# orottier/web-audio-api-rs

Measured on NVIDIA H100. Metric: offline render-quanta/sec (48kHz stereo, 128-frame), higher is better.
Workload: dtype f64 filter state / f32 PCM

## Files before the change

web-audio-api-rs_b200/csrc/wae_engine.cu:

```cuda
#include "wae_graph.h"
#include "wae_hostmath.h"
#include "wae_hrtf_host.h"
#include "wae_resample_host.h"
#include "wae_kernels.h"
#include "wae_param_core.h"
#include "wae_param_host.h"

#include <cuda_runtime.h>
#include <emmintrin.h>

#include <algorithm>
#include <atomic>
#include <chrono>
#include <condition_variable>
#include <cstdlib>
#include <deque>
#include <fstream>
#include <mutex>
#include <sched.h>
#include <sstream>
#include <thread>
#include <cmath>
#include <cstdio>
#include <cstring>
// ... 576 lines not shown
    Node* n = nullptr;
    int level = 0;
    std::vector<std::vector<PortRef>> in_edges;
    std::vector<int> in_ch;
    std::vector<BufRef> in_buf;
    std::vector<Lay> in_lay;
    std::vector<int> out_ch;
    std::vector<BufRef> out_buf;
    std::vector<Lay> out_lay;
    bool wrote_dest = false;
    Lay lay_out(int port) const { return port < (int)out_lay.size() ? out_lay[port] : Lay::fixed(out_ch[port]); }
};

struct NodeTable {
    std::vector<PNode> v;
    std::vector<char> has;
    void reset(uint32_t max_id) {
        if (v.size() < (size_t)max_id + 1) v.resize((size_t)max_id + 1);
        has.assign(v.size(), 0);
    }
    PNode& put(uint32_t id, Node* n) {
        if (id >= v.size()) {
            v.resize((size_t)id + 1);
            has.resize((size_t)id + 1, 0);
        }
        PNode& p = v[id];
        p.n = n;
        p.level = 0;
        p.in_edges.resize((size_t)n->n_inputs);
        for (auto& port : p.in_edges) port.clear();
        p.in_ch.clear();
        p.in_buf.clear();
        p.in_lay.clear();
        p.out_ch.clear();
        p.out_buf.clear();
        p.out_lay.clear();
        p.wrote_dest = false;
        has[id] = 1;
        return p;
    }
    PNode* find(uint32_t id) { return id < v.size() && has[id] ? &v[id] : nullptr; }
    bool count(uint32_t id) const { return id < v.size() && has[id]; }
    PNode& at(uint32_t id) {
        if (!(id < v.size() && has[id])) throw std::out_of_range("planner: unknown node id");
        return v[id];
    }
};

struct Planner {
    wae_batch* b;
    wae_engine* eng;
    std::map<std::pair<int, int>, StageBuild> builds;
    std::string error;
    int error_code = 0;
    uint64_t algorithmic_bytes = 0;
    struct IrSpectra {
        float2* h;
        int S;
        int channels;
    };
    std::unordered_map<uint64_t, IrSpectra> own_ir_cache;
    std::unordered_map<uint64_t, IrSpectra>* ir_cache = &own_ir_cache;
    std::map<int, std::pair<const float2*, const float2*>> os_filters;

    bool has_feedback = false;
    std::map<std::pair<uint32_t, uint32_t>, int>* delay_ch_hint = nullptr;
    std::map<std::pair<uint32_t, uint32_t>, int> delay_ch_seen;
    struct DelayRing {
        float* ring;
        uint32_t ring_len;
        int ch;
        int64_t* mono_at;
        int32_t mono_len;
    };
    std::map<std::pair<uint32_t, uint32_t>, DelayRing> delay_rings;
    std::map<std::pair<uint32_t, uint32_t>, int> conv_paths_seen;
    bool dry = false;
    int group_graphs = 1;
    int vs_mode = -1;
    int voice_sum_mode() {
        if (eng->voice_sum >= 0) return eng->voice_sum;
        if (vs_mode < 0) {
            const char* e = getenv("WAE_VOICE_SUM");
            vs_mode = e ? std::max(0, std::min(2, atoi(e))) : 0;
        }
        return vs_mode;
    }
    uint64_t arena_floats_per_frame = 0;
    float* d_src = nullptr;
    std::vector<wae_batch::Group::SrcCopy>* src_copies = nullptr;
    size_t src_cursor = 0;
    struct PendingChain {
        ChainInst inst;
        hm::BiquadCoefs coefs[CHAIN_MAX_BIQUADS] = {};
        int ch = 1;
        int phase = 0;
        int cls = 0;
        Lay lay;
    };

    uint32_t key_graph = 0, key_node = 0, key_seq = 0;
    uint64_t key_salt = 0;
    template <typename T>
    T* alloc(size_t count, bool zero = false, bool rezero_on_run = false) {
        if (dry) return reinterpret_cast<T*>(uintptr_t(256));
        if (seg_start == 0 && seg_end >= lq) return b->dalloc<T>(count, zero, rezero_on_run);
        const wae_batch::StateKey key{key_graph, key_node, key_seq++, key_salt};
        const size_t bytes = count * sizeof(T);
        std::lock_guard<std::recursive_mutex> lk(b->mu);
        auto it = b->state_map.find(key);
        if (it != b->state_map.end() && it->second.second == bytes) return (T*)it->second.first;
        T* p = b->dalloc<T>(count, zero, rezero_on_run);
        if (p) b->state_map[key] = {(void*)p, bytes};
        return p;
    }
    std::map<int, std::vector<float*>> arena_pool;
    std::map<int, size_t> arena_used;
    std::map<std::pair<uint32_t, uint32_t>, size_t> src_offsets;
    std::unordered_map<const PcmBuffer*, size_t> buf_offsets;
    struct ParamRecord {
        size_t n_source_events = 0;
        ParamTimeline tl;
        int64_t init_frame = 0;
    };
    std::unordered_map<uint64_t, ParamRecord> param_records;
    const ParamTimeline* param_timeline(uint32_t gi, uint32_t pid, const Param& prm, float sample_rate) {
        const uint64_t rec_key = (uint64_t)gi << 32 | pid;
        auto it = param_records.find(rec_key);
        if (it == param_records.end()) {
            ParamRecord r;
            r.tl = build_param_timeline(prm);
            r.n_source_events = prm.events.size();
            r.init_frame = seg_start;
            return &param_records.emplace(rec_key, std::move(r)).first->second.tl;
        }
        ParamRecord& r = it->second;
        if (r.n_source_events == prm.events.size() || !r.tl.error.empty()) return &r.tl;
        ParamInst host{};
        host.events = r.tl.events.data();
        host.curves = r.tl.curves.data();
        host.n_events = (int32_t)r.tl.events.size();
        host.a_rate = prm.a_rate ? 1 : 0;
        host.sample_rate = sample_rate;
        ParamState st{};
        st.intrinsic = r.tl.intrinsic;
        st.has_last = r.tl.has_last ? 1 : 0;
        st.last = r.tl.last;
        st.inited = 1;
        float buf[128];
        for (int64_t f = r.init_frame; f < seg_start; f += 128) param_compute_buffer(host, st, (double)f / (double)sample_rate, buf);
        ParamTimeline next;
        next.curves = r.tl.curves;
        for (int i = st.head; i < host.n_events; i++) next.events.push_back(i == st.head && st.override_valid ? st.override_ev : r.tl.events[i]);
        next.intrinsic = st.intrinsic;
        next.has_last = st.has_last != 0;
        next.last = st.last;
        fold_param_events(next, prm.events.data() + r.n_source_events, prm.events.size() - r.n_source_events);
        r.tl = std::move(next);
        r.n_source_events = prm.events.size();
        r.init_frame = seg_start;
        return &r.tl;
    }
    int64_t seg_start = 0, seg_end = 0;
    int64_t lq = 0, glq = 0;
    BufRef dest_ref(const wae_graph* g, uint32_t gi) const { return BufRef{b->d_out + b->out_off[gi], (uint32_t)g->length, 1}; }
    void begin_segment(int64_t f0, int64_t f1) {
        seg_start = f0;
// ... 593 lines not shown
                    m.n_edges = (int)edges.size();
                    m.edge_offset = (uint32_t)ms.mix_edges.size();
                    m.limit = -1;
                    for (auto& r : edges) ms.mix_edges.push_back(MixEdge{pn.at(r.node).out_buf[r.port], pn.at(r.node).out_ch[r.port], 0});
                    ms.mix_dyn.push_back(m);
                    pi.in = m.out;
                } else {
                    StageBuild& ms = stage(2 * level, S_MIX);
                    MixInst m{};
                    m.out = arena_buf(1);
                    if (!m.out.p) return bail(WAE_OUT_OF_MEMORY, "out of device memory (arena)");
                    m.out_ch = 1;
                    m.interp = WAE_INTERPRETATION_DISCRETE;
                    m.n_edges = (int)edges.size();
                    m.edge_offset = (uint32_t)ms.mix_edges.size();
                    m.limit = -1;
                    for (auto& r : edges) ms.mix_edges.push_back(MixEdge{pn.at(r.node).out_buf[r.port], pn.at(r.node).out_ch[r.port], 0});
                    ms.mix.push_back(m);
                    pi.in = m.out;
                }
            }
            pi.events = tl.events.empty() ? nullptr : upload(tl.events);
            pi.curves = tl.curves.empty() ? nullptr : upload(tl.curves);
            pi.state = alloc<ParamState>(1, true, true);
            pi.out = arena_buf(2);
            if (!pi.state || !pi.out.p) return bail(WAE_OUT_OF_MEMORY, "out of device memory (param)");
            pi.def = n.param.default_value;
            pi.mn = n.param.min_value;
            pi.mx = n.param.max_value;
            pi.intrinsic0 = tl.intrinsic;
            pi.has_last0 = tl.has_last ? 1 : 0;
            pi.last0 = tl.last;
            pi.sample_rate = g->sample_rate;
            pi.n_events = (int32_t)tl.events.size();
            pi.a_rate = n.param.a_rate ? 1 : 0;
            stage(2 * level + 1, S_PARAM).param.push_back(pi);
            p.out_ch = {1};
            p.out_buf = {pi.out};
            continue;
        }
        int level = 0;
        for (auto& port : p.in_edges)
            for (auto& r : port) level = std::max(level, pn.at(r.node).level + 1);
        bool dyn_params = false;
        for (uint32_t pid : n.params) {
            PNode& pp = pn.at(pid);
            if (!pp.out_buf.empty()) {
                dyn_params = true;
                level = std::max(level, pp.level + 1);
            }
        }
        if (n.kind == K_PANNER)
            for (uint32_t pid = 2; pid <= 10; pid++)
                if (pn.count(pid) && !pn.at(pid).out_buf.empty()) level = std::max(level, pn.at(pid).level + 1);
        p.level = level;
        const bool fuse_n = fuse && !dyn_params;
        uint32_t fuse_src = 0;
        bool extend = false, dest_direct = false;
        const bool chain_kind = !dyn_params && ((n.kind == K_BIQUAD && !eng->serial_filters) || (fuse && (n.kind == K_GAIN || (n.kind == K_SHAPER && !(n.oversample && n.has_curve)))));
        if (fuse && n.n_inputs == 1 && p.in_edges[0].size() == 1 && p.in_edges[0][0].port == 0) {
            auto it = pending.find(p.in_edges[0][0].node);
            if (it != pending.end()) {
                int sch = pn.at(it->first).out_ch[0];
                if (chain_kind && computed_channels(n.cfg, sch) == sch && chain_accepts(it->second, n.kind)) {
                    extend = true;
                    fuse_src = it->first;
                } else if (n.kind == K_DEST && g->length <= 0xffffffffull &&
                           (sch == (int)g->channels || (sch == 1 && g->channels == 2 && n.cfg.interp == WAE_INTERPRETATION_SPEAKERS))) {
                    dest_direct = true;
                    fuse_src = it->first;
                }
            }
        }
        std::vector<char> port_vsum(p.in_edges.size(), 0);
        std::vector<int> port_vsum_nb(p.in_edges.size(), 0);
        if (fuse && voice_sum_mode() != 0 && !extend && !dest_direct && cur_cls == 0 && n.kind != K_DELAY_R) {
            for (size_t pi = 0; pi < p.in_edges.size() && (int)pi < n.n_inputs; pi++) {
                const auto& edges = p.in_edges[pi];
                if ((int)edges.size() < 8) continue;
                const int ch = computed_channels(n.cfg, 1);
                if (!(ch == 1 || (ch == 2 && n.cfg.interp == WAE_INTERPRETATION_SPEAKERS))) continue;
                if (n.kind == K_DEST && g->length > 0xffffffffull) continue;
                const int64_t tiles = (seg_end - seg_start + 2047) / 2048;
                if (voice_sum_mode() < 2 && tiles * (int64_t)group_graphs < 2 * (int64_t)voice_sum_slots()) continue;
                int nb = -1;
                bool ok = true;
                std::set<uint32_t> seen_nodes;
                for (auto& r : edges) {
                    auto it = pending.find(r.node);
                    if (r.port != 0 || it == pending.end()) { ok = false; break; }
                    const PendingChain& pc = it->second;
                    if (pc.inst.src_kind != CHAIN_SRC_OSC || pc.ch != 1 || pc.inst.has_shaper || pc.inst.n_biquad > 1 || pc.lay.dyn() || pc.cls != cur_cls ||
                        (nb >= 0 && nb != pc.inst.n_biquad) || !seen_nodes.insert(r.node).second) { ok = false; break; }
                    nb = pc.inst.n_biquad;
                }
                if (!ok) continue;
                port_vsum[pi] = 1;
                port_vsum_nb[pi] = nb;
            }
        }
        for (size_t pi = 0; pi < p.in_edges.size(); pi++) {
            if (port_vsum[pi]) continue;
            auto& port = p.in_edges[pi];
            for (auto& r : port)
                if (!((extend || dest_direct) && r.node == fuse_src))
                    if (!materialize(r.node, n.kind == K_CONV && n.buffer && port.size() == 1)) return false;
        }
        p.in_ch.assign(n.n_inputs, 1);
        p.in_buf.assign(n.n_inputs, BufRef{nullptr, 0, 0});
        p.in_lay.assign(n.n_inputs, Lay::fixed(1));
        for (int port = 0; port < n.n_inputs; port++) {
            auto& edges = p.in_edges[port];
            int max_in = 1;
            for (auto& r : edges) max_in = std::max(max_in, pn.at(r.node).out_ch[r.port]);
            int ch = computed_channels(n.cfg, max_in);
            if (n.kind == K_DELAY_R) {
                ch = max_in;
            }
            p.in_ch[port] = ch;
            p.in_lay[port] = Lay::fixed(ch);
            bool is_dest = n.kind == K_DEST;
            if (extend || dest_direct) {
                if (extend) p.in_lay[port] = pending.at(fuse_src).lay;
                continue;
            }
            if (port_vsum[port]) {
                StageBuild& vs = stage(2 * level, S_VSUM, port_vsum_nb[port]);
                VoiceGroup vg{};
                vg.first = (int32_t)vs.chain.size();
                vg.n_voices = (int32_t)edges.size();
                vg.out_dup = ch;
                vg.limit = -1;
                if (is_dest) {
                    vg.out = dest_ref(g, gi);
                    vg.limit = (int64_t)g->length;
                } else {
                    vg.out = arena_buf(ch);
                    if (!vg.out.p) return bail(WAE_OUT_OF_MEMORY, "out of device memory (arena)");
                }
                for (auto& r : edges) {
                    PendingChain pc = std::move(pending.at(r.node));
                    pending.erase(r.node);
                    if (pc.inst.n_biquad == 1 && vs.n_scan_coef != vs.chain.size()) return bail(WAE_UNSUPPORTED, "internal: voice-sum coefficient table out of step");
                    for (int k = 0; k < pc.inst.n_biquad; k++)
                        pc.inst.bq[k].coef = vs.add_scan_coef(want_scan_coefs, [&] { return make_scan_coef(pc.coefs[k]); });
                    pc.inst.limit = -1;
                    pc.inst.out_dup = 0;
                    vs.chain.push_back(pc.inst);
                }
                vs.vgroups.push_back(vg);
                p.in_buf[port] = vg.out;
                continue;
            }
            if (is_dest && edges.size() == 1 && pn.at(edges[0].node).wrote_dest) {
                p.in_buf[port] = pn.at(edges[0].node).out_buf[edges[0].port];
                continue;
            }
            bool any_dyn = false;
            Lay pl = Lay::fixed(ch);
            if (!edges.empty()) {
                int lo = 1, hi = 1, on_nlo = 0, min_nlo = 255;
                bool all_may_silent = true;
                for (auto& r : edges) {
                    const Lay el = pn.at(r.node).lay_out(r.port);
                    any_dyn = any_dyn || el.dyn();
                    lo = std::max<int>(lo, el.lo);
                    hi = std::max<int>(hi, el.hi);
// ... 1149 lines not shown
    CUDA_TRY(cudaStreamCreateWithFlags(&eng->s_d2h, cudaStreamNonBlocking));
    if (const char* e = getenv("WAE_BIND_NUMA"))
        if (atoi(e) != 0) bind_to_device_numa_node(eng);
    std::vector<float> sine = hm::sine_table();
    CUDA_TRY(cudaMalloc(&eng->d_sine, sine.size() * sizeof(float)));
    CUDA_TRY(cudaMemcpy(eng->d_sine, sine.data(), sine.size() * sizeof(float), cudaMemcpyHostToDevice));
    upload_twiddles();
    CUDA_TRY(cudaDeviceSynchronize());
    *out = eng;
    return WAE_OK;
}

WAE_API wae_status wae_engine_destroy(wae_engine* eng) {
    if (!eng) return WAE_OK;
    cudaSetDevice(eng->device);
    if (eng->d_sine) cudaFree(eng->d_sine);
    if (eng->d_sphere_ir) cudaFree(eng->d_sphere_ir);
    if (eng->d_sphere_pos) cudaFree(eng->d_sphere_pos);
    if (eng->d_sphere_tri) cudaFree(eng->d_sphere_tri);
    eng->drop_rate_spheres();
    delete eng->sphere;
    delete eng->pool;
    eng->dev_trim();
    for (int i = 0; i < wae_engine::kStageSlots; i++)
        if (eng->h_stage[i]) cudaFreeHost(eng->h_stage[i]);
    if (eng->h_ring) cudaFreeHost(eng->h_ring);
    if (eng->stream) cudaStreamDestroy(eng->stream);
    if (eng->s_h2d) cudaStreamDestroy(eng->s_h2d);
    if (eng->s_d2h) cudaStreamDestroy(eng->s_d2h);
    delete eng;
    return WAE_OK;
}

WAE_API wae_status wae_engine_set_hrir_sphere(wae_engine* eng, const void* data, uint64_t len) {
    if (!eng) return fail(WAE_INVALID_ARGUMENT, "null engine");
    auto* sp = new HrirSphere();
    std::string err;
    if (!sp->parse(static_cast<const uint8_t*>(data), len, err)) {
        delete sp;
        return fail(WAE_INVALID_ARGUMENT, err.c_str());
    }
    CUDA_TRY(cudaSetDevice(eng->device));
    float* d = nullptr;
    if (cudaMalloc(&d, sp->ir.size() * sizeof(float)) != cudaSuccess) {
        delete sp;
        return fail(WAE_OUT_OF_MEMORY, "out of device memory (HRIR sphere)");
    }
    float* dpos = nullptr;
    uint32_t* dtri = nullptr;
    if (cudaMalloc(&dpos, sp->pos.size() * sizeof(float)) != cudaSuccess || cudaMalloc(&dtri, sp->tri.size() * sizeof(uint32_t)) != cudaSuccess) {
        cudaFree(d);
        if (dpos) cudaFree(dpos);
        delete sp;
        return fail(WAE_OUT_OF_MEMORY, "out of device memory (HRIR sphere)");
    }
    cudaMemcpy(d, sp->ir.data(), sp->ir.size() * sizeof(float), cudaMemcpyHostToDevice);
    cudaMemcpy(dpos, sp->pos.data(), sp->pos.size() * sizeof(float), cudaMemcpyHostToDevice);
    cudaMemcpy(dtri, sp->tri.data(), sp->tri.size() * sizeof(uint32_t), cudaMemcpyHostToDevice);
    CUDA_TRY(cudaStreamSynchronize(eng->stream));
    if (eng->d_sphere_ir) cudaFree(eng->d_sphere_ir);
    if (eng->d_sphere_pos) cudaFree(eng->d_sphere_pos);
    if (eng->d_sphere_tri) cudaFree(eng->d_sphere_tri);
    eng->drop_rate_spheres();
    eng->d_sphere_pos = dpos;
    eng->d_sphere_tri = dtri;
    delete eng->sphere;
    eng->sphere = sp;
    eng->d_sphere_ir = d;
    return WAE_OK;
}

WAE_API wae_status wae_engine_stream(wae_engine* eng, void** out_stream) {
    *out_stream = (void*)eng->stream;
    return WAE_OK;
}

WAE_API wae_status wae_engine_set_option(wae_engine* eng, uint32_t option, int64_t value) {
    switch (option) {
        case WAE_OPT_CHUNK_FRAMES:
            if (value < 0 || value % 128 != 0) return fail(WAE_INVALID_ARGUMENT, "chunk frames must be a multiple of 128");
            eng->chunk_frames = value;
            return WAE_OK;
        case WAE_OPT_FUSE: eng->fuse = value != 0; return WAE_OK;
        case WAE_OPT_VOICE_SUM: eng->voice_sum = value < 0 ? 0 : (value > 2 ? 2 : (int)value); return WAE_OK;
        case WAE_OPT_SERIAL_FILTERS: eng->serial_filters = value != 0; return WAE_OK;
        case WAE_OPT_PIPELINE_GROUPS:
            if (value < 0 || value > 1024) return fail(WAE_INVALID_ARGUMENT, "pipeline groups must be in [0, 1024]");
            eng->pipeline_groups = (int)value;
            return WAE_OK;
        case WAE_OPT_PARAM_PARALLEL: eng->param_parallel = value > 2 ? 2 : (int)value; return WAE_OK;
        case WAE_OPT_BIND_NUMA:
            if (value != 0 && eng->pool) return fail(WAE_INVALID_STATE, "bind the engine to its NUMA node before its first render (worker threads already run)");
            if (value != 0 && !bind_to_device_numa_node(eng)) return fail(WAE_UNSUPPORTED, "could not read / apply the CPU list of the GPU's NUMA node");
            return WAE_OK;
        case WAE_OPT_HOST_WORKERS:
            if (value < 0 || value > 256) return fail(WAE_INVALID_ARGUMENT, "host workers must be in [0, 256]");
            if (eng->pool) return fail(WAE_INVALID_STATE, "the worker threads already run");
            eng->n_workers = (int)value;
            return WAE_OK;
        case WAE_OPT_CHAIN_TMA: chain_set_tuning(value != 0 ? 1 : 0, -1); return WAE_OK;
        case WAE_OPT_CHAIN_WAVES:
            if (value < 0 || value > 1024) return fail(WAE_INVALID_ARGUMENT, "chain waves must be in [0, 1024]");
            chain_set_tuning(-1, (int)value);
            return WAE_OK;
        case WAE_OPT_CHAIN_PREPASS: chain_set_prepass(value != 0 ? 1 : 0); return WAE_OK;
        default: return fail(WAE_INVALID_ARGUMENT, "unknown option");
    }
}

WAE_API wae_status wae_batch_destroy(wae_batch* b) {
    if (!b) return WAE_OK;
    cudaSetDevice(b->engine->device);
    if (b->engine->stream) {
        cudaStreamSynchronize(b->engine->stream);
        cudaStreamSynchronize(b->engine->s_h2d);
        cudaStreamSynchronize(b->engine->s_d2h);
    }
    for (void* h : b->pinned) cudaFreeHost(h);
    for (auto& g : b->groups) {
        if (g.ev_h2d) cudaEventDestroy(g.ev_h2d);
        if (g.ev_done) cudaEventDestroy(g.ev_done);
    }
    for (void* p : b->allocs) b->engine->dev_release(p);
    if (b->ev0) cudaEventDestroy(b->ev0);
    if (b->ev1) cudaEventDestroy(b->ev1);
    for (auto e : b->stage_events) cudaEventDestroy(e);
    delete b;
    return WAE_OK;
}

WAE_API wae_status wae_graph_render_order(wae_graph* g, wae_node_id* ids, uint32_t cap, uint32_t* n) {
    if (!g || !n || (cap && !ids)) return fail(WAE_INVALID_ARGUMENT, "null argument");
    Orderer o;
    o.g = g;
    o.run();
    *n = (uint32_t)o.ordered.size();
    for (uint32_t i = 0; i < *n && i < cap; i++) ids[i] = o.ordered[i];
    return WAE_OK;
}

struct PrepState {
    std::map<std::pair<uint32_t, uint32_t>, int> delay_ch_hint;
    std::unordered_map<uint64_t, Planner::IrSpectra> ir_cache;
    uint64_t algorithmic_bytes = 0;
    std::chrono::steady_clock::time_point t0, t1;
};
struct GroupPlan {
    std::vector<Stage> stages;
    std::vector<std::pair<size_t, size_t>> seg_ranges;
    uint64_t algorithmic_bytes = 0;
    int code = WAE_OK;
    std::string error;
};

static int64_t padded_length(const wae_graph* g) { return (int64_t)((g->length + 127) / 128 * 128); }

static std::vector<int64_t> graph_cuts(const wae_graph* g) {
    const int64_t lq = padded_length(g);
    std::vector<int64_t> cuts;
    for (auto& ep : g->epochs)
        if ((int64_t)ep.frame > 0 && (int64_t)ep.frame < lq) cuts.push_back((int64_t)ep.frame);
    return cuts;
}

constexpr int64_t kGroupPadNum = 3, kGroupPadDen = 4;
static bool fits_group(int64_t longest, int64_t lq) { return lq * kGroupPadDen >= longest * kGroupPadNum; }

// ... 1500 lines not shown
```

web-audio-api-rs_b200/csrc/wae_kernels.cu:

```cuda
#include "wae_kernels.h"
#include "wae_param_core.h"
#include "wae_param_walk.h"
#include "../../include/wae.h"

#include <algorithm>
#include <cmath>
#include <cstdlib>
#include <vector>
#include <type_traits>
#include <cuda_runtime.h>
#include <math_constants.h>

namespace wae {

#define DEVI __device__ __forceinline__

DEVI float* chan(const BufRef& b, int c, const ChunkInfo& ci) { return b.p + (size_t)c * b.stride + (b.absolute ? ci.f0 : ci.sub); }

DEVI int meta_qi(const ChunkInfo& ci, int n) { return (ci.sub + n) >> 7; }
DEVI bool buf_silent(const BufRef& b, int rows, int qi) {
    if (!b.meta) return false;
    for (int r = 0; r < rows; r++)
        if (!(b.meta[(size_t)r * b.meta_stride + qi] & WAE_META_SILENT)) return false;
    return true;
// ... 882 lines not shown
                unsigned mask = 0;
                if (type == 2) {
                    const unsigned long long cw = HALF + dph;
#pragma unroll
                    for (int j = 0; j < CH_K; j++) {
                        v[j] = __ll2float_rn((long long)ph) * 1.08420217248550443e-19f;
                        if ((unsigned)((ph + cw) >> 32) <= thr) mask |= 1u << j;
                        asm("add.u64 %0, %0, %1;" : "+l"(ph) : "l"(dph));
                    }
                    while (mask) {
                        const int jw = __ffs((int)mask) - 1;
                        mask &= mask - 1;
                        const unsigned long long pj = ph0 + (unsigned long long)jw * dph;
                        const float sw = osc_saw_blep(pj + HALF, inc, inv);
#pragma unroll
                        for (int j = 0; j < CH_K; j++) v[j] = j == jw ? sw : v[j];
                    }
                } else {
                    const bool wide = dph >= 0x4000000000000000ull;
#pragma unroll
                    for (int j = 0; j < CH_K; j++) {
                        v[j] = (long long)ph >= 0 ? 1.0f : -1.0f;
                        if (((unsigned)((ph + dph) >> 32) & 0x7fffffffu) <= thr) mask |= 1u << j;
                        asm("add.u64 %0, %0, %1;" : "+l"(ph) : "l"(dph));
                    }
                    if (wide) mask = (1u << CH_K) - 1u;
                    while (mask) {
                        const int jw = __ffs((int)mask) - 1;
                        mask &= mask - 1;
                        const unsigned long long pj = ph0 + (unsigned long long)jw * dph;
                        const float sw = osc_square_blep(pj, pj + HALF, inc, inv);
#pragma unroll
                        for (int j = 0; j < CH_K; j++) v[j] = j == jw ? sw : v[j];
                    }
                }
            } else {
#pragma unroll
                for (int j = 0; j < CH_K; j++) {
                    long long q = (long long)(ph - 0x4000000000000000ull);
                    q = q < 0 ? -q : q;
                    v[j] = __ll2float_rn((long long)(0x4000000000000000ull - (unsigned long long)q)) * 2.16840434497100887e-19f;
                    asm("add.u64 %0, %0, %1;" : "+l"(ph) : "l"(dph));
                }
            }
        } else {
#pragma unroll
            for (int j = 0; j < CH_K; j++) {
                int64_t n = na + j;
                float s = 0.f;
                if (n >= o.n_first && n < o.n_stop && !o.outside_nyquist) s = osc_sample(o, osc_phase_at(o, n), o.incr);
                v[j] = s;
            }
        }
    } else {
        const ConstInst& o = q.cst;
#pragma unroll
        for (int j = 0; j < CH_K; j++) {
            int64_t n = ci.f0 + n0 + j;
            v[j] = (n >= o.n_first && n < o.n_stop) ? o.value : 0.f;
        }
    }
}

template <int SRC>
__device__ __noinline__ void chain_stage_gather(const ChainInst* q, int c, ChunkInfo ci, int n0, float4* region, int lane, int xq) {
    float tmp[CH_K];
    chain_load_source<SRC>(*q, c, ci, n0, tmp);
#pragma unroll
    for (int u = 0; u < CH_K / 4; u++) region[4 * lane + (u ^ xq)] = make_float4(tmp[4 * u], tmp[4 * u + 1], tmp[4 * u + 2], tmp[4 * u + 3]);
}

struct ChainSmem {
    ChainInst q;
    double state[CHAIN_MAX_BIQUADS][4];
    double P[CHAIN_MAX_BIQUADS][24];
    double plane[CHAIN_MAX_BIQUADS][32][4];
    double wtot[CH_WARPS][2];
    double replay[4];
    float edge[CH_WARPS][2];
    int flushed;
};

struct NoReload {};
template <typename RL>
DEVI void chain_biquad(ChainSmem& sm, int bq, const double b0, const double b1, const double b2, const double a1, const double a2,
                       const double* Plane, float v[CH_K], bool active, int n_active, int t, int lane, int warp, bool want_clean, bool& clean,
                       RL reload) {
    const double* Psh = sm.P[bq];
    const double* Pw = sm.P[bq] + 20;
    const float xl1 = active ? v[CH_K - 1] : 0.f, xl2 = active ? v[CH_K - 2] : 0.f;
    if (lane == 31) {
        sm.edge[warp][0] = xl1;
        sm.edge[warp][1] = xl2;
    }
    const float p1 = __shfl_up_sync(0xffffffffu, xl1, 1);
    const float p2 = __shfl_up_sync(0xffffffffu, xl2, 1);
    __syncthreads();
    double x1, x2;
    if (lane == 0) {
        if (warp == 0) {
            x1 = sm.state[bq][0];
            x2 = sm.state[bq][1];
        } else {
            x1 = (double)sm.edge[warp - 1][0];
            x2 = (double)sm.edge[warp - 1][1];
        }
    } else {
        x1 = (double)p1;
        x2 = (double)p2;
    }
    const bool x_normal = want_clean && (isnormal_d(x1) || isnormal_d(x2));
    double w[CH_K];
    double r1 = 0., r2 = 0.;
    const double na1 = -a1, na2 = -a2;
#pragma unroll
    for (int j = 0; j < CH_K; j++) {
        const double x = (double)v[j];
        w[j] = fma(b2, x2, fma(b1, x1, b0 * x));
        const double y = fma(na1, r1, fma(na2, r2, w[j]));
        x2 = x1;
        x1 = x;
        r2 = r1;
        r1 = y;
    }
    double va = active ? r1 : 0., vb = active ? r2 : 0.;
#pragma unroll
    for (int d = 0; d < 5; d++) {
        const double oa = __shfl_up_sync(0xffffffffu, va, 1 << d);
        const double ob = __shfl_up_sync(0xffffffffu, vb, 1 << d);
        if (lane >= (1 << d)) mat2_fma(Psh + 4 * d, oa, ob, va, vb);
    }
    if (lane == 31) {
        sm.wtot[warp][0] = va;
        sm.wtot[warp][1] = vb;
    }
    const double ea = __shfl_up_sync(0xffffffffu, va, 1);
    const double eb = __shfl_up_sync(0xffffffffu, vb, 1);
    __syncthreads();
    double wa = sm.state[bq][2], wb = sm.state[bq][3];
#pragma unroll
    for (int k = 0; k < CH_WARPS - 1; k++) {
        if (k < warp) {
            double ta = sm.wtot[k][0], tb = sm.wtot[k][1];
            mat2_fma(Pw, wa, wb, ta, tb);
            wa = ta;
            wb = tb;
        }
    }
    double e1 = wa, e2 = wb;
    if (lane != 0) {
        e1 = ea;
        e2 = eb;
        mat2_fma(Plane, wa, wb, e1, e2);
    }
    if (want_clean) clean = !(x_normal || isnormal_d(e1) || isnormal_d(e2));
    r1 = e1;
    r2 = e2;
#pragma unroll
    for (int j = 0; j < CH_K; j++) {
        const double y = fma(na1, r1, fma(na2, r2, w[j]));
        r2 = r1;
        r1 = y;
        v[j] = (float)y;
    }
    const bool last = active && t == n_active - 1;
    const bool poisoned = last && (!(fabs(r1) <= 1.7976931348623157e308) || !(fabs(r2) <= 1.7976931348623157e308));
#ifdef WAE_CHAIN_NOCHECK
    __syncthreads();
    if (false) {
#else
    if (__syncthreads_or(poisoned)) {
#endif
        if (t == 0) sm.flushed = 1;
        if constexpr (!std::is_same<RL, NoReload>::value) {
            float x[CH_K];
            reload(x);
            double sx1 = sm.state[bq][0], sx2 = sm.state[bq][1], sy1 = sm.state[bq][2], sy2 = sm.state[bq][3];
            __syncthreads();
#pragma unroll 1
            for (int wv = 0; wv < CH_WARPS; wv++) {
                if (warp == wv) {
#pragma unroll 1
                    for (int l = 0; l < 32; l++) {
                        double qx1 = sx1, qx2 = sx2, qy1 = sy1, qy2 = sy2;
                        if (lane == l && active) {
#pragma unroll
                            for (int j = 0; j < CH_K; j++) {
                                const double xi = (double)x[j];
                                double y = __dsub_rn(__dsub_rn(__dadd_rn(__dadd_rn(__dmul_rn(b0, xi), __dmul_rn(b1, qx1)), __dmul_rn(b2, qx2)), __dmul_rn(a1, qy1)),
                                                     __dmul_rn(a2, qy2));
                                if (!isnormal_d(y)) y = 0.;
                                qx2 = qx1;
                                qx1 = xi;
                                qy2 = qy1;
                                qy1 = y;
                                v[j] = (float)y;
                            }
                        }
                        sx1 = __shfl_sync(0xffffffffu, qx1, l);
                        sx2 = __shfl_sync(0xffffffffu, qx2, l);
                        sy1 = __shfl_sync(0xffffffffu, qy1, l);
                        sy2 = __shfl_sync(0xffffffffu, qy2, l);
                    }
                    if (lane == 0) {
                        sm.replay[0] = sx1;
                        sm.replay[1] = sx2;
                        sm.replay[2] = sy1;
                        sm.replay[3] = sy2;
                    }
                }
                __syncthreads();
                sx1 = sm.replay[0];
                sx2 = sm.replay[1];
                sy1 = sm.replay[2];
                sy2 = sm.replay[3];
                __syncthreads();
            }
            if (t == 0) {
                sm.state[bq][0] = sx1;
                sm.state[bq][1] = sx2;
// ... 494 lines not shown
    __shared__ ChainSmem sm;
    __shared__ int s_item;
    __shared__ float2 s_table2[2048];
    const int t = threadIdx.x, lane = t & 31, warp = t >> 5;
    if (t == 0) {
        const unsigned tk = atomicAdd(sc.ticket, 1u);
        if (tk == gridDim.x - 1) atomicExch(sc.ticket, 0u);
        s_item = (int)tk;
    }
    __syncthreads();
    const int item = s_item;
    const int slab = item / n_groups, gi = item - slab * n_groups;
    const VoiceGroup grp = groups[gi];
    constexpr int tile = CH_THREADS * CH_K;
    const int base = slab * tile;
    if (base >= ci.nf) return;
    const int n0 = base + t * CH_K;
    const bool active = n0 < ci.nf;
    const int n_active = min(CH_THREADS, (ci.nf - base) / CH_K);
    const bool first_slab = slab == 0, last_slab = base + tile >= ci.nf;
    const unsigned tag = (sc.epoch & 0xfffu) << 20;
    const unsigned* prog_prev = sc.flags + (size_t)gi * sc.slab_stride + (slab > 0 ? slab - 1 : 0);
    unsigned* prog_mine = sc.flags + (size_t)gi * sc.slab_stride + slab;
    unsigned seen = 0;
    const float* cur_table = nullptr;
    float acc[CH_K];
#pragma unroll
    for (int j = 0; j < CH_K; j++) acc[j] = 0.f;
    constexpr int REC_W = (int)(sizeof(ChainInst) / 4 + CH_THREADS - 1) / CH_THREADS;
    constexpr int PL_W = (128 + CH_THREADS - 1) / CH_THREADS;
    static_assert(CH_THREADS >= 24, "scan constants: one of Pshfl / Pwarp per thread");
    int rec_n[REC_W];
    double pl_n[PL_W], pw_n = 0.;
    auto prefetch = [&](int vi) {
        const int inst = grp.first + vi;
        const int* src = reinterpret_cast<const int*>(insts + inst);
#pragma unroll
        for (int i = 0; i < REC_W; i++) rec_n[i] = (t + i * CH_THREADS) < (int)(sizeof(ChainInst) / 4) ? __ldg(src + t + i * CH_THREADS) : 0;
        if (NB > 0) {
            const ScanCoef& scf = coefs[inst];
#pragma unroll
            for (int i = 0; i < PL_W; i++) pl_n[i] = (t + i * CH_THREADS) < 128 ? (&scf.Plane[0][0])[t + i * CH_THREADS] : 0.;
            if (t < 20) pw_n = (&scf.Pshfl[0][0])[t];
            else if (t < 24) pw_n = scf.Pwarp[t - 20];
        }
    };
    prefetch(0);
    const bool handoff_in = NB > 0 && !first_slab, handoff_out = NB > 0 && !last_slab;
    auto poll_ok = [&](unsigned x, int v) { return (x & 0xfff00000u) == tag && (x & 0xfffffu) > (unsigned)v; };
    double st_next = 0.;
    bool st_next_valid = false;
    constexpr int PUB_T = CH_WARPS > 1 ? 32 : 0;
    double pe0 = 0., pe1 = 0., pe2 = 0., pe3 = 0.;
    double* pub_ptr = nullptr;
    int pub_vi = -1;
    auto publish = [&]() {
        if (pub_vi < 0) return;
        if (last_slab) {
            pub_ptr[0] = pe0; pub_ptr[1] = pe1; pub_ptr[2] = pe2; pub_ptr[3] = pe3;
        } else {
            double* dst = sc.handoff + ((size_t)(grp.first + pub_vi) * 2 + ((slab + 1) & 1)) * 4;
            asm volatile("st.global.cg.v2.f64 [%0], {%1, %2};" ::"l"(dst), "d"(pe0), "d"(pe1) : "memory");
            asm volatile("st.global.cg.v2.f64 [%0], {%1, %2};" ::"l"(dst + 2), "d"(pe2), "d"(pe3) : "memory");
            asm volatile("st.release.gpu.global.u32 [%0], %1;" ::"l"(prog_mine), "r"(tag | (unsigned)(pub_vi + 1)) : "memory");
        }
        pub_vi = -1;
    };
    for (int vi = 0; vi < grp.n_voices; vi++) {
        const int inst = grp.first + vi;
#pragma unroll
        for (int i = 0; i < REC_W; i++)
            if ((t + i * CH_THREADS) < (int)(sizeof(ChainInst) / 4)) reinterpret_cast<int*>(&sm.q)[t + i * CH_THREADS] = rec_n[i];
        if (NB > 0) {
#pragma unroll
            for (int i = 0; i < PL_W; i++)
                if ((t + i * CH_THREADS) < 128) (&sm.plane[0][0][0])[t + i * CH_THREADS] = pl_n[i];
            if (t < 24) sm.P[0][t] = pw_n;
        }
        __syncthreads();
        if (vi + 1 < grp.n_voices) prefetch(vi + 1);
        const ChainInst& q = sm.q;
        double st_cur = 0.;
        unsigned xa = 0;
        if (NB > 0 && t == PUB_T) publish();
        if (NB > 0 && warp == 0) {
            if (st_next_valid) {
                st_cur = st_next;
            } else if (first_slab) {
                if (lane < 4) st_cur = q.bq[0].state[lane];
            } else {
                if (lane == 0 && seen <= (unsigned)vi) {
                    for (;;) {
                        unsigned x;
                        asm volatile("ld.relaxed.gpu.global.u32 %0, [%1];" : "=r"(x) : "l"(prog_prev) : "memory");
                        if (poll_ok(x, vi)) {
                            seen = x & 0xfffffu;
                            break;
                        }
                        __nanosleep(20);
                    }
                }
                __syncwarp();
                if (lane < 4) st_cur = __ldcg(sc.handoff + ((size_t)inst * 2 + (slab & 1)) * 4 + lane);
            }
            if (handoff_in && lane == 0 && vi + 1 < grp.n_voices && seen <= (unsigned)(vi + 1))
                asm volatile("ld.relaxed.gpu.global.u32 %0, [%1];" : "=r"(xa) : "l"(prog_prev));
        }
        const float2* tab2 = nullptr;
        if ((q.osc.type == 0 || q.osc.type == 4) && q.osc.table_len == 2048) {
            if (q.osc.table != cur_table) {
                const float* gt = q.osc.table;
                for (int i = t; i < 2048; i += CH_THREADS) s_table2[i] = make_float2(__ldg(gt + i), __ldg(gt + ((i + 1) & 2047)));
                cur_table = gt;
                __syncthreads();
            }
            tab2 = s_table2;
        }
        double cb[5] = {0., 0., 0., 0., 0.};
        double* st_ptr = nullptr;
        if (NB > 0) {
            const ChainBiquad& bq = q.bq[0];
            cb[0] = bq.b0; cb[1] = bq.b1; cb[2] = bq.b2; cb[3] = bq.a1; cb[4] = bq.a2;
            st_ptr = bq.state;
        }
        const float g0 = q.g[0], g1 = q.g[1];
        float v[CH_K];
        if (active) chain_load_source<CHAIN_SRC_OSC>(q, 0, ci, n0, v, tab2);
        if (g0 != 1.f) {
#pragma unroll
            for (int j = 0; j < CH_K; j++) v[j] *= g0;
        }
        if (NB > 0) {
            if (warp == 0 && lane < 4) sm.state[0][lane] = st_cur;
            bool clean = true;
            chain_biquad(sm, 0, cb[0], cb[1], cb[2], cb[3], cb[4], sm.plane[0][lane > 0 ? lane - 1 : 0], v, active, n_active, t, lane, warp, false, clean, NoReload{});
            if (g1 != 1.f) {
#pragma unroll
                for (int j = 0; j < CH_K; j++) v[j] *= g1;
            }
        }
        if (active) {
            if (vi == 0) {
#pragma unroll
                for (int j = 0; j < CH_K; j++) acc[j] = v[j];
            } else {
#pragma unroll
                for (int j = 0; j < CH_K; j++) acc[j] += v[j];
            }
        }
        if (NB > 0 && first_slab && warp == 0) {
            st_next_valid = vi + 1 < grp.n_voices;
            if (st_next_valid && lane < 4) st_next = insts[inst + 1].bq[0].state[lane];
        }
        if (handoff_in && warp == 0) {
            st_next_valid = false;
            if (vi + 1 < grp.n_voices) {
                if (lane == 0 && seen <= (unsigned)(vi + 1) && poll_ok(xa, vi + 1)) seen = xa & 0xfffffu;
                st_next_valid = __shfl_sync(0xffffffffu, seen > (unsigned)(vi + 1) ? 1 : 0, 0) != 0;
                if (st_next_valid && lane < 4) st_next = __ldcg(sc.handoff + ((size_t)(inst + 1) * 2 + (slab & 1)) * 4 + lane);
            }
        }
        __syncthreads();
        if (NB > 0 && t == PUB_T) {
            pe0 = sm.state[0][0]; pe1 = sm.state[0][1]; pe2 = sm.state[0][2]; pe3 = sm.state[0][3];
            pub_ptr = st_ptr;
            pub_vi = vi;
        }
    }
    if (NB > 0 && t == PUB_T) publish();
    (void)handoff_out;
    if (!active) return;
    const int64_t nabs = ci.f0 + n0;
    for (int oc = 0; oc < grp.out_dup; oc++) {
        float* out = chan(grp.out, oc, ci) + n0;
        if ((reinterpret_cast<uintptr_t>(out) & 15) == 0 && (grp.limit < 0 || nabs + CH_K <= grp.limit)) {
#pragma unroll
            for (int u = 0; u < CH_K / 4; u++) reinterpret_cast<float4*>(out)[u] = make_float4(acc[4 * u], acc[4 * u + 1], acc[4 * u + 2], acc[4 * u + 3]);
        } else {
#pragma unroll
            for (int j = 0; j < CH_K; j++)
                if (grp.limit < 0 || nabs + j < grp.limit) out[j] = acc[j];
        }
    }
}

__global__ void __launch_bounds__(256) k_osc_arate(const OscArInst* __restrict__ insts, int n_inst, ChunkInfo ci) {
    __shared__ double s_sum[256];
    __shared__ double s_carry;
    const OscArInst q = insts[blockIdx.x];
    const OscInst& o = q.base;
    float* out = chan(o.out, 0, ci);
    const float* ft = q.freq.p ? chan(q.freq, 0, ci) : nullptr;
    const float* dtk = q.detune.p ? chan(q.detune, 0, ci) : nullptr;
    const int t = threadIdx.x;
    const double sr = (double)q.sample_rate, nyq = sr / 2.;
    if (t == 0) s_carry = *q.phase;
    __syncthreads();
    for (int base = 0; base < ci.nf; base += 2048) {
        const int n0 = base + t * 8;
        double inc[8];
        bool act[8], oob[8];
        double local = 0.;
#pragma unroll
        for (int j = 0; j < 8; j++) {
            const int n = n0 + j;
            const int64_t na = ci.f0 + n;
            act[j] = n < ci.nf && na >= o.n_first && na < o.n_stop;
            double cf = 0.;
            if (n < ci.nf) {
                float f = ft ? ft[n] : q.f_val, d = dtk ? dtk[n] : q.d_val;
                cf = (double)f * exp2((double)d / 1200.);
            }
            oob[j] = fabs(cf) >= nyq;
            inc[j] = cf / sr;
            double add = act[j] ? inc[j] : 0.;
            if (act[j] && na == o.n_first) add += q.start_ratio * inc[j];
            local += add;
        }
// ... 2411 lines not shown
```

Measured before the change: 1.400 billion.

## Defer voice-sum state handoff wait until biquad needs it; enable new default mode

In the voice-sum chain kernel, the wait on the previous slab's progress flag and the load of its handed-over biquad state move into a hook that runs inside chain_biquad, just before the state is read. The x-history terms are recomputed locally from the oscillator source, so the spin-wait can overlap the local scan work. The default voice-sum mode also changes from off to a new mode 3, which turns the fused voice-sum path on by default with a heuristic based on tile count and voice count. This may cost extra oscillator evaluation per voice, and it carries correctness risk in the state split and in the handoff prefetch condition.

```diff
diff --git a/web-audio-api-rs_b200/csrc/wae_engine.cu b/web-audio-api-rs_b200/csrc/wae_engine.cu
--- a/web-audio-api-rs_b200/csrc/wae_engine.cu
+++ b/web-audio-api-rs_b200/csrc/wae_engine.cu
@@ -682,7 +682,7 @@
         if (eng->voice_sum >= 0) return eng->voice_sum;
         if (vs_mode < 0) {
             const char* e = getenv("WAE_VOICE_SUM");
-            vs_mode = e ? std::max(0, std::min(2, atoi(e))) : 0;
+            vs_mode = e ? std::max(0, std::min(2, atoi(e))) : 3;
         }
         return vs_mode;
     }
@@ -1442,7 +1442,8 @@
                 if (!(ch == 1 || (ch == 2 && n.cfg.interp == WAE_INTERPRETATION_SPEAKERS))) continue;
                 if (n.kind == K_DEST && g->length > 0xffffffffull) continue;
                 const int64_t tiles = (seg_end - seg_start + 2047) / 2048;
-                if (voice_sum_mode() < 2 && tiles * (int64_t)group_graphs < 2 * (int64_t)voice_sum_slots()) continue;
+                if (voice_sum_mode() != 2 && tiles * (int64_t)group_graphs < 2 * (int64_t)voice_sum_slots()) continue;
+                if (voice_sum_mode() == 3 && std::min<int64_t>(tiles, (int64_t)edges.size()) * group_graphs < 2 * (int64_t)voice_sum_slots()) continue;
                 int nb = -1;
                 bool ok = true;
                 std::set<uint32_t> seen_nodes;
@@ -2758,7 +2759,7 @@
             eng->chunk_frames = value;
             return WAE_OK;
         case WAE_OPT_FUSE: eng->fuse = value != 0; return WAE_OK;
-        case WAE_OPT_VOICE_SUM: eng->voice_sum = value < 0 ? 0 : (value > 2 ? 2 : (int)value); return WAE_OK;
+        case WAE_OPT_VOICE_SUM: eng->voice_sum = value < 0 ? -1 : (value > 2 ? 2 : (int)value); return WAE_OK;
         case WAE_OPT_SERIAL_FILTERS: eng->serial_filters = value != 0; return WAE_OK;
         case WAE_OPT_PIPELINE_GROUPS:
             if (value < 0 || value > 1024) return fail(WAE_INVALID_ARGUMENT, "pipeline groups must be in [0, 1024]");
diff --git a/web-audio-api-rs_b200/csrc/wae_kernels.cu b/web-audio-api-rs_b200/csrc/wae_kernels.cu
--- a/web-audio-api-rs_b200/csrc/wae_kernels.cu
+++ b/web-audio-api-rs_b200/csrc/wae_kernels.cu
@@ -988,10 +988,13 @@
 };
 
 struct NoReload {};
-template <typename RL>
+struct NoHook {
+    DEVI void operator()() const {}
+};
+template <typename RL, typename PB = NoHook>
 DEVI void chain_biquad(ChainSmem& sm, int bq, const double b0, const double b1, const double b2, const double a1, const double a2,
                        const double* Plane, float v[CH_K], bool active, int n_active, int t, int lane, int warp, bool want_clean, bool& clean,
-                       RL reload) {
+                       RL reload, PB pre_state = PB{}) {
     const double* Psh = sm.P[bq];
     const double* Pw = sm.P[bq] + 20;
     const float xl1 = active ? v[CH_K - 1] : 0.f, xl2 = active ? v[CH_K - 2] : 0.f;
@@ -1042,6 +1045,7 @@
     }
     const double ea = __shfl_up_sync(0xffffffffu, va, 1);
     const double eb = __shfl_up_sync(0xffffffffu, vb, 1);
+    pre_state();
     __syncthreads();
     double wa = sm.state[bq][2], wb = sm.state[bq][3];
 #pragma unroll
@@ -1702,28 +1706,15 @@
         const ChainInst& q = sm.q;
         double st_cur = 0.;
         unsigned xa = 0;
+        const bool st_known = st_next_valid || first_slab;
         if (NB > 0 && t == PUB_T) publish();
         if (NB > 0 && warp == 0) {
             if (st_next_valid) {
                 st_cur = st_next;
             } else if (first_slab) {
                 if (lane < 4) st_cur = q.bq[0].state[lane];
-            } else {
-                if (lane == 0 && seen <= (unsigned)vi) {
-                    for (;;) {
-                        unsigned x;
-                        asm volatile("ld.relaxed.gpu.global.u32 %0, [%1];" : "=r"(x) : "l"(prog_prev) : "memory");
-                        if (poll_ok(x, vi)) {
-                            seen = x & 0xfffffu;
-                            break;
-                        }
-                        __nanosleep(20);
-                    }
-                }
-                __syncwarp();
-                if (lane < 4) st_cur = __ldcg(sc.handoff + ((size_t)inst * 2 + (slab & 1)) * 4 + lane);
-            }
-            if (handoff_in && lane == 0 && vi + 1 < grp.n_voices && seen <= (unsigned)(vi + 1))
+            }
+            if (handoff_in && lane == 0 && seen <= (unsigned)(vi + 1))
                 asm volatile("ld.relaxed.gpu.global.u32 %0, [%1];" : "=r"(xa) : "l"(prog_prev));
         }
         const float2* tab2 = nullptr;
@@ -1751,9 +1742,43 @@
             for (int j = 0; j < CH_K; j++) v[j] *= g0;
         }
         if (NB > 0) {
-            if (warp == 0 && lane < 4) sm.state[0][lane] = st_cur;
+            if (warp == 0) {
+                if (st_known) {
+                    if (lane < 4) sm.state[0][lane] = st_cur;
+                } else if (lane == 0) {
+                    float h[CH_K];
+                    chain_load_source<CHAIN_SRC_OSC>(q, 0, ci, base - CH_K, h, tab2);
+                    if (g0 != 1.f) {
+                        h[CH_K - 1] *= g0;
+                        h[CH_K - 2] *= g0;
+                    }
+                    sm.state[0][0] = (double)h[CH_K - 1];
+                    sm.state[0][1] = (double)h[CH_K - 2];
+                }
+            }
+            auto hand_over = [&]() {
+                if (st_known || warp != 0) return;
+                if (lane == 0 && seen <= (unsigned)vi) {
+                    if (poll_ok(xa, vi)) {
+                        seen = xa & 0xfffffu;
+                    } else {
+                        for (;;) {
+                            unsigned x;
+                            asm volatile("ld.relaxed.gpu.global.u32 %0, [%1];" : "=r"(x) : "l"(prog_prev) : "memory");
+                            if (poll_ok(x, vi)) {
+                                seen = x & 0xfffffu;
+                                break;
+                            }
+                            __nanosleep(20);
+                        }
+                    }
+                }
+                __syncwarp();
+                if (lane == 2 || lane == 3) sm.state[0][lane] = __ldcg(sc.handoff + ((size_t)inst * 2 + (slab & 1)) * 4 + lane);
+            };
             bool clean = true;
-            chain_biquad(sm, 0, cb[0], cb[1], cb[2], cb[3], cb[4], sm.plane[0][lane > 0 ? lane - 1 : 0], v, active, n_active, t, lane, warp, false, clean, NoReload{});
+            chain_biquad(sm, 0, cb[0], cb[1], cb[2], cb[3], cb[4], sm.plane[0][lane > 0 ? lane - 1 : 0], v, active, n_active, t, lane, warp, false, clean, NoReload{},
+                         hand_over);
             if (g1 != 1.f) {
 #pragma unroll
                 for (int j = 0; j < CH_K; j++) v[j] *= g1;
```

Result: no change. 1.401 billion, median of 6 (+0.1%).
